# LuoweiZhou/VLP

Measured on NVIDIA H100. Metric: image_text_samples_per_sec, higher is better.
Workload: dtype bf16

## Files before the change

### vlp_b200/csrc/api.cu

```cuda
#include "../../include/vlpk.h"

#include <cstdlib>
#include <cstring>

#include "attn.cuh"
#include "decode.cuh"
#include "gemm.cuh"
#include "head.cuh"
#include "host.cuh"
#include "optim.cuh"
#include "rowops.cuh"
#include "tables.cuh"

using namespace vlpk;
typedef __nv_bfloat16 bf16;

namespace {

inline cudaStream_t S(void* s) { return reinterpret_cast<cudaStream_t>(s); }

enum { SITE_ATTN = 0, SITE_HID1 = 1, SITE_HID2 = 2 };
inline uint64_t site_of(uint64_t layer_id, int site) { return layer_id * 8 + site; }

inline DropoutCfg mk_drop(const VlpkDropout* d, float p, uint64_t site) {
// ... 322 lines not shown
  const long long i = (static_cast<long long>(blockIdx.x) * blockDim.x + threadIdx.x) * 8;
  if (i >= M * N) return;
  const long long r = i / N;
  const int c = static_cast<int>(i % N);
  const uint4 ud = *reinterpret_cast<const uint4*>(dy + r * lddy + c), uy = *reinterpret_cast<const uint4*>(y + r * ldy + c);
  const uint32_t wd[4] = {ud.x, ud.y, ud.z, ud.w}, wy[4] = {uy.x, uy.y, uy.z, uy.w};
  uint32_t o[4];
#pragma unroll
  for (int j = 0; j < 4; ++j) {
    const float2 d = unpack_bf16x2(wd[j]), v = unpack_bf16x2(wy[j]);
    o[j] = pack_bf16x2(v.x > 0.f ? d.x * scale : 0.f, v.y > 0.f ? d.y * scale : 0.f);
  }
  *reinterpret_cast<uint4*>(dpre + i) = make_uint4(o[0], o[1], o[2], o[3]);
}

int score_layer_fwd(const VlpkShape* s, int T, const AttnGroupKv* group, const VlpkLayerWeights* w, const void* x, const uint32_t* key_bits,
                    const uint32_t* query_bits, VlpkLayerActs* a, uint64_t layer_id, cudaStream_t st) {
  const int H = s->H, K = group != nullptr ? T - 1 : s->Lq, R = K + T;
  VLPK_TRY(qkv_fwd(s->B * R, H, w, x, a->qkv, st));
  const bf16* qkv = static_cast<const bf16*>(a->qkv);
  AttnGroupKv g;
  if (group != nullptr) {
    g = *group;
    g.text = qkv + H; g.ld_text = 3 * H; g.T = R; g.pos = 0;
  }
  AttnDesc ad;
  ad.B = s->B; ad.heads = s->heads; ad.Lkv = s->Lkv; ad.kv_slots = s->kv_slots;
  ad.q = qkv; ad.ld_q = 3 * H; ad.q_batch_stride = static_cast<int64_t>(R) * 3 * H;
  ad.k = qkv + H; ad.v = qkv + 2 * H; ad.kv_batch_stride = static_cast<int64_t>(R) * 3 * H;
  ad.ld_kv = group != nullptr ? 2 * H : 3 * H;
  ad.o = a->ctx; ad.ld_o = H; ad.o_batch_stride = static_cast<int64_t>(R) * H;
  ad.lse = a->lse;
  ad.drop = make_dropout(0.f, 0, 0);
  if (K > 0) {
    AttnDesc kd = ad;
    kd.Lq = K;
    kd.mask_bits = key_bits; kd.mask_rows = K;
    VLPK_TRY(launch_attn_fwd(kd, group != nullptr ? &g : nullptr, nullptr, st));
  }
  AttnDesc qd = ad;
  qd.Lq = T;
  qd.q = qkv + static_cast<size_t>(K) * 3 * H;
  qd.o = static_cast<bf16*>(a->ctx) + static_cast<size_t>(K) * H;
  qd.mask_bits = query_bits; qd.mask_rows = T;
  qd.lse = a->lse + static_cast<size_t>(s->B) * s->heads * K;
  AttnSelfKv sk;
  sk.k = qkv + static_cast<size_t>(K) * 3 * H + H;
  sk.v = qkv + static_cast<size_t>(K) * 3 * H + 2 * H;
  sk.ld = 3 * H; sk.batch_stride = static_cast<int64_t>(R) * 3 * H;
  VLPK_TRY(launch_attn_fwd(qd, group != nullptr ? &g : nullptr, &sk, st));
  VlpkShape rows = *s;
  rows.Lq = rows.Lkv = R;
  VLPK_TRY(attn_out_ln(&rows, w, x, a, 0.f, nullptr, layer_id, st));
  return ffn_fwd_impl(&rows, w, a, 0.f, nullptr, layer_id, st);
}

int score_stack_fwd(const VlpkShape* s, int T, int n_layers, const VlpkLayerWeights* w, const void* x, AttnGroupKv* group,
                    const void* const* prefix, const uint32_t* key_bits, const uint32_t* query_bits, VlpkLayerActs* acts, cudaStream_t st) {
  const void* cur = x;
  for (int i = 0; i < n_layers; ++i) {
    if (group != nullptr) group->prefix = prefix[i];
    VLPK_TRY(score_layer_fwd(s, T, group, &w[i], cur, key_bits, query_bits, &acts[i], i, st));
    cur = acts[i].y;
  }
  return 0;
}

size_t act_bytes(const VlpkShape* s, size_t rows, size_t kv_elems) {
  const size_t H = s->H, I = s->I, M = static_cast<size_t>(s->B) * rows;
  const size_t lse = (static_cast<size_t>(s->B) * s->heads * rows + 3) / 4 * 4;
  return 2 * (M * (3 * H + 5 * H + 2 * I) + kv_elems) + 4 * (lse + 4 * M);
}

}

#pragma GCC visibility push(default)
extern "C" {

int vlpk_version(void) { return VLPK_VERSION; }
int vlpk_debug_set_option(const char* name, int value) {
  VLPK_CHECK_ARG(name != nullptr, "set_option: null name");
  if (strcmp(name, "wgrad_stream") == 0) { g_wgrad_stream = value ? 1 : 0; return 0; }
  if (strcmp(name, "attn_tiled") == 0) { set_attn_tiled(value != 0); return 0; }
  set_error("set_option: unknown option '%s'", name);
  return -1;
}
int vlpk_debug_plan_gemm(int M, int N, int K, int a_mn, int b_mn, int nseg, int seg_rows, int epi, int bn, int splits, int* out2) {
  GemmDesc g;
  g.M = M; g.N = N; g.K = K;
  g.a_mn = a_mn != 0; g.b_mn = b_mn != 0;
  g.nseg = nseg; g.b_seg_rows = seg_rows;
  g.epi = epi; g.bn = bn; g.splits = splits;
  return plan_gemm(g, &out2[0], &out2[1]);
}
void vlpk_set_reserved_sms(int n) { set_reserved_sms(n); }
void vlpk_set_deterministic(int on) { set_deterministic(on != 0); }
const char* vlpk_last_error(void) { return get_error(); }

int vlpk_mask_pack(const void* mask, int dtype, int mode, int B, int rows, int kv, int64_t stride_b, int64_t stride_r, uint32_t* out,
                   void* stream) {
  VLPK_CHECK_ARG(mask != nullptr && out != nullptr, "mask_pack: null pointer");
  return launch_mask_pack(mask, dtype, mode, B, rows, kv, stride_b, stride_r, out, S(stream));
}

int vlpk_mask_synth(const int32_t* len_b, const int32_t* mode, int len_a, int B, int L, uint32_t* out, void* stream) {
  return launch_mask_synth(len_b, mode, len_a, B, L, out, S(stream));
}

int vlpk_linear_fwd(int M, int N, int K, const void* x, int64_t ldx, const void* w, int64_t ldw, const void* bias, void* y, int64_t ldy,
                    int act, const VlpkDropout* drop, uint64_t site, void* stream) {
  VLPK_CHECK_ARG(x && w && y, "linear_fwd: null pointer");
  VLPK_CHECK_ARG(act == VLPK_ACT_NONE || act == VLPK_ACT_RELU, "linear_fwd: act %d unsupported", act);
  const DropoutCfg dc = (act == VLPK_ACT_RELU && drop != nullptr) ? mk_drop(drop, drop->p, site) : make_dropout(0.f, 0, site);
  return fwd_linear(M, N, K, x, ldx, w, ldw, bias, y, ldy, act == VLPK_ACT_RELU ? EPI_RELU : EPI_STORE, nullptr, 0, dc, S(stream));
}

int vlpk_linear_bwd(int M, int N, int K, const void* x, int64_t ldx, const void* w, int64_t ldw, const void* y, int64_t ldy,
                    const void* dy, int64_t lddy, void* dpre, void* dx, int64_t lddx, float* dw, int64_t lddw, float* db, int act,
                    float p_drop, void* stream) {
  VLPK_CHECK_ARG(x && w && dy && dw, "linear_bwd: null pointer");
  cudaStream_t st = S(stream);
  const void* g = dy;
  int64_t ldg = lddy;
  if (act == VLPK_ACT_RELU) {
    VLPK_CHECK_ARG(y != nullptr && dpre != nullptr && N % 8 == 0, "linear_bwd: relu needs y, dpre and N %% 8 == 0");
    const long long n = static_cast<long long>(M) * N;
    LaunchScope scope(CAT_MISC, 6.0 * n, st);
    relu_bwd_kernel<<<static_cast<unsigned>((n / 8 + 255) / 256), 256, 0, st>>>(static_cast<bf16*>(dpre), static_cast<const bf16*>(dy),
                                                                             static_cast<const bf16*>(y), M, N, lddy, ldy,
                                                                             p_drop > 0.f ? 1.0f / (1.0f - p_drop) : 1.0f);
    VLPK_CUDA(cudaGetLastError());
    g = dpre;
    ldg = N;
  }
  if (db != nullptr) VLPK_TRY(launch_colsum(g, ldg, M, N, db, st));
  VLPK_TRY(wgrad_linear(M, N, K, g, ldg, x, ldx, dw, lddw, st));
  if (dx != nullptr) VLPK_TRY(dgrad_linear(M, N, K, g, ldg, w, ldw, dx, lddx, EPI_STORE, nullptr, 0, st));
  return 0;
}

static EmbedArgs mk_embed(int B, int L, int H, int R, int vis_input, const int64_t* ids, const int64_t* tt, const int64_t* pos,
                          const void* word_w, const void* pos_w, const void* type_w, const void* vis, const void* vpe,
                          const void* ln_g) {
  EmbedArgs a;
  a.B = B; a.L = L; a.H = H; a.R = R; a.vis_input = vis_input;
  a.ids = reinterpret_cast<const long long*>(ids);
  a.tt = reinterpret_cast<const long long*>(tt);
  a.pos = reinterpret_cast<const long long*>(pos);
  a.word = static_cast<const bf16*>(word_w); a.posw = static_cast<const bf16*>(pos_w); a.typew = static_cast<const bf16*>(type_w);
  a.vis = static_cast<const bf16*>(vis); a.vpe = static_cast<const bf16*>(vpe);
  a.gamma = static_cast<const bf16*>(ln_g);
  return a;
}

int vlpk_embed_fwd(int B, int L, int H, int R, int vis_input, const int64_t* ids, const int64_t* token_type, const int64_t* pos,
                   const void* word_w, const void* pos_w, const void* type_w, const void* vis, const void* vis_pe, const void* ln_g,
                   const void* ln_b, void* y, float* stats, const VlpkDropout* drop, uint64_t site, void* stream) {
  VLPK_CHECK_ARG(ids && word_w && pos_w && type_w && ln_g && ln_b && y, "embed_fwd: null pointer");
  EmbedArgs a = mk_embed(B, L, H, R, vis_input, ids, token_type, pos, word_w, pos_w, type_w, vis, vis_pe, ln_g);
  a.beta = static_cast<const bf16*>(ln_b);
  a.y = static_cast<bf16*>(y);
  a.stats = reinterpret_cast<float2*>(stats);
  a.drop = mk_drop(drop, drop ? drop->p : 0.f, site);
  return launch_embed_fwd(a, S(stream));
}

// ... 476 lines not shown
```

### vlp_b200/csrc/common.cuh

```cuda
#pragma once
#include <cuda.h>
#include <cuda_bf16.h>
#include <cuda_runtime.h>
#include <stdint.h>

#include "wgmma.cuh"

namespace vlpk {

__device__ __forceinline__ uint32_t smem_u32(const void* p) {
  return static_cast<uint32_t>(__cvta_generic_to_shared(p));
}

__device__ __forceinline__ uint32_t lane_id() { return threadIdx.x & 31u; }

__device__ __forceinline__ bool elect_one() {
  uint32_t pred = 0;
  asm volatile(
      "{\n\t"
      ".reg .pred P;\n\t"
      "elect.sync _|P, 0xffffffff;\n\t"
      "selp.u32 %0, 1, 0, P;\n\t"
      "}\n"
      : "=r"(pred));
// ... 4 lines not shown
  asm volatile("mbarrier.init.shared::cta.b64 [%0], %1;" ::"r"(smem_u32(bar)), "r"(count) : "memory");
}
__device__ __forceinline__ void fence_mbar_init() {
  asm volatile("fence.mbarrier_init.release.cluster;" ::: "memory");
}
__device__ __forceinline__ void fence_proxy_async_smem() {
  asm volatile("fence.proxy.async.shared::cta;" ::: "memory");
}
__device__ __forceinline__ void mbar_arrive_expect_tx(uint64_t* bar, uint32_t bytes) {
  asm volatile("mbarrier.arrive.expect_tx.shared::cta.b64 _, [%0], %1;" ::"r"(smem_u32(bar)), "r"(bytes)
               : "memory");
}
__device__ __forceinline__ void mbar_arrive(uint64_t* bar) {
  asm volatile("mbarrier.arrive.shared::cta.b64 _, [%0];" ::"r"(smem_u32(bar)) : "memory");
}
__device__ __forceinline__ bool mbar_try_wait(uint64_t* bar, uint32_t parity) {
  uint32_t ok;
  asm volatile(
      "{\n\t"
      ".reg .pred P;\n\t"
      "mbarrier.try_wait.parity.shared::cta.b64 P, [%1], %2;\n\t"
      "selp.u32 %0, 1, 0, P;\n\t"
      "}\n"
      : "=r"(ok)
      : "r"(smem_u32(bar)), "r"(parity)
      : "memory");
  return ok != 0;
}
__device__ __forceinline__ void mbar_wait(uint64_t* bar, uint32_t parity) {
  uint32_t spins = 0;
  while (!mbar_try_wait(bar, parity)) {
    if (++spins > (1u << 28)) { __trap(); }
  }
}
__device__ __forceinline__ void mbar_wait_flag(uint64_t* bar, uint32_t parity, bool& timed_out) {
  uint32_t spins = 0;
  while (!timed_out && !mbar_try_wait(bar, parity)) {
    if (++spins > (1u << 28)) timed_out = true;
  }
}

__device__ __forceinline__ void pdl_launch_dependents() { asm volatile("griddepcontrol.launch_dependents;" ::: "memory"); }
__device__ __forceinline__ void pdl_wait() { asm volatile("griddepcontrol.wait;" ::: "memory"); }

__device__ __forceinline__ void tma_prefetch_desc(const CUtensorMap* m) {
  asm volatile("prefetch.tensormap [%0];" ::"l"(reinterpret_cast<uint64_t>(m)) : "memory");
}
__device__ __forceinline__ void tma_load_2d(void* dst, const CUtensorMap* m, uint64_t* bar, int c0, int c1) {
  asm volatile(
      "cp.async.bulk.tensor.2d.shared::cluster.global.tile.mbarrier::complete_tx::bytes [%0], [%1, {%3, %4}], [%2];"
      ::"r"(smem_u32(dst)), "l"(reinterpret_cast<uint64_t>(m)), "r"(smem_u32(bar)), "r"(c0), "r"(c1)
      : "memory");
}
__device__ __forceinline__ void tma_load_3d(void* dst, const CUtensorMap* m, uint64_t* bar, int c0, int c1,
                                            int c2) {
  asm volatile(
      "cp.async.bulk.tensor.3d.shared::cluster.global.tile.mbarrier::complete_tx::bytes [%0], [%1, {%3, %4, %5}], "
      "[%2];" ::"r"(smem_u32(dst)),
      "l"(reinterpret_cast<uint64_t>(m)), "r"(smem_u32(bar)), "r"(c0), "r"(c1), "r"(c2)
      : "memory");
}
__device__ __forceinline__ void tma_store_2d(const CUtensorMap* m, const void* src, int c0, int c1) {
  asm volatile("cp.async.bulk.tensor.2d.global.shared::cta.tile.bulk_group [%0, {%2, %3}], [%1];" ::"l"(
                   reinterpret_cast<uint64_t>(m)),
               "r"(smem_u32(src)), "r"(c0), "r"(c1)
               : "memory");
}
__device__ __forceinline__ void tma_store_3d(const CUtensorMap* m, const void* src, int c0, int c1, int c2) {
  asm volatile("cp.async.bulk.tensor.3d.global.shared::cta.tile.bulk_group [%0, {%2, %3, %4}], [%1];" ::"l"(
                   reinterpret_cast<uint64_t>(m)),
               "r"(smem_u32(src)), "r"(c0), "r"(c1), "r"(c2)
               : "memory");
}
__device__ __forceinline__ void tma_reduce_add_2d(const CUtensorMap* m, const void* src, int c0, int c1) {
  asm volatile("cp.reduce.async.bulk.tensor.2d.global.shared::cta.add.tile.bulk_group [%0, {%2, %3}], [%1];" ::"l"(
                   reinterpret_cast<uint64_t>(m)),
               "r"(smem_u32(src)), "r"(c0), "r"(c1)
               : "memory");
}
__device__ __forceinline__ void tma_reduce_add_3d(const CUtensorMap* m, const void* src, int c0, int c1, int c2) {
  asm volatile("cp.reduce.async.bulk.tensor.3d.global.shared::cta.add.tile.bulk_group [%0, {%2, %3, %4}], [%1];" ::"l"(
                   reinterpret_cast<uint64_t>(m)),
               "r"(smem_u32(src)), "r"(c0), "r"(c1), "r"(c2)
               : "memory");
}
__device__ __forceinline__ void tma_store_commit() { asm volatile("cp.async.bulk.commit_group;" ::: "memory"); }
template <int N>
__device__ __forceinline__ void tma_store_wait_read() {
  asm volatile("cp.async.bulk.wait_group.read %0;" ::"n"(N) : "memory");
}
template <int N>
__device__ __forceinline__ void tma_store_wait() {
  asm volatile("cp.async.bulk.wait_group %0;" ::"n"(N) : "memory");
}

__device__ __forceinline__ void wgmma_fence() { asm volatile("wgmma.fence.sync.aligned;" ::: "memory"); }
__device__ __forceinline__ void wgmma_commit() { asm volatile("wgmma.commit_group.sync.aligned;" ::: "memory"); }
template <int N>
__device__ __forceinline__ void wgmma_wait() {
  asm volatile("wgmma.wait_group.sync.aligned %0;" ::"n"(N) : "memory");
}
template <uint32_t N>
__device__ __forceinline__ void setmaxnreg_dec() { asm volatile("setmaxnreg.dec.sync.aligned.u32 %0;" ::"n"(N)); }
template <uint32_t N>
__device__ __forceinline__ void setmaxnreg_inc() { asm volatile("setmaxnreg.inc.sync.aligned.u32 %0;" ::"n"(N)); }
template <int N>
__device__ __forceinline__ void reg_fence(float (&d)[N]) {
#pragma unroll
  for (int i = 0; i < N; ++i) asm volatile("" : "+f"(d[i])::"memory");
}

__device__ __forceinline__ uint64_t wgmma_desc_sw128(uint32_t saddr, uint32_t lbo_bytes, uint32_t sbo_bytes) {
  uint64_t d = 0;
  d |= static_cast<uint64_t>((saddr & 0x3FFFFu) >> 4);
  d |= static_cast<uint64_t>((lbo_bytes >> 4) & 0x3FFFu) << 16;
  d |= static_cast<uint64_t>((sbo_bytes >> 4) & 0x3FFFu) << 32;
  d |= 1ull << 62;
  return d;
}

__device__ __forceinline__ uint32_t pack_bf16x2(float lo, float hi) {
  __nv_bfloat162 v = __floats2bfloat162_rn(lo, hi);
  return *reinterpret_cast<uint32_t*>(&v);
}
__device__ __forceinline__ float2 unpack_bf16x2(uint32_t u) {
  __nv_bfloat162 v = *reinterpret_cast<__nv_bfloat162*>(&u);
  return __bfloat1622float2(v);
}
__device__ __forceinline__ float bf16_round(float x) { return __bfloat162float(__float2bfloat16_rn(x)); }

__device__ __forceinline__ float fast_ex2(float x) {
  float y;
  asm("ex2.approx.ftz.f32 %0, %1;" : "=f"(y) : "f"(x));
  return y;
}
__device__ __forceinline__ float fast_rcp(float x) {
  float y;
  asm("rcp.approx.ftz.f32 %0, %1;" : "=f"(y) : "f"(x));
  return y;
}

__device__ __forceinline__ void gelu_and_grad(float x, float& g, float& d) {
  const float ax = fabsf(x);
  const float e = fast_ex2(-0.72134752044448170f * x * x);
  const float t = fast_rcp(fmaf(0.3275911f * 0.70710678118654752f, ax, 1.0f));
  float poly = fmaf(1.061405429f, t, -1.453152027f);
  poly = fmaf(poly, t, 1.421413741f);
  poly = fmaf(poly, t, -0.284496736f);
  poly = fmaf(poly, t, 0.254829592f);
  poly *= t;
  const float erf_abs = fmaf(-poly, e, 1.0f);
  const float cdf = 0.5f * (1.0f + copysignf(erf_abs, x));
  g = x * cdf;
  d = fmaf(x * 0.3989422804014327f, e, cdf);
}

struct Philox {
  __device__ __forceinline__ static uint4 gen(uint64_t seed, uint64_t ctr_hi, uint64_t ctr_lo) {
    uint32_t k0 = static_cast<uint32_t>(seed), k1 = static_cast<uint32_t>(seed >> 32);
    uint4 c = make_uint4(static_cast<uint32_t>(ctr_lo), static_cast<uint32_t>(ctr_lo >> 32),
                         static_cast<uint32_t>(ctr_hi), static_cast<uint32_t>(ctr_hi >> 32));
#pragma unroll
    for (int i = 0; i < 10; ++i) {
      const uint32_t hi0 = __umulhi(0xD2511F53u, c.x), lo0 = 0xD2511F53u * c.x;
      const uint32_t hi1 = __umulhi(0xCD9E8D57u, c.z), lo1 = 0xCD9E8D57u * c.z;
      c = make_uint4(hi1 ^ c.y ^ k0, lo1, hi0 ^ c.w ^ k1, lo0);
// ... 49 lines not shown
```

### vlp_b200/csrc/rowops.cu

```cuda
#include "rowops.cuh"

#include <cstdlib>
#include "host.cuh"

namespace vlpk {

static constexpr int MAXCH = 4;

__device__ __forceinline__ float warp_sum(float v) {
#pragma unroll
  for (int o = 16; o > 0; o >>= 1) v += __shfl_xor_sync(0xffffffffu, v, o);
  return v;
}

__device__ __forceinline__ void load8(const __nv_bfloat16* p, float (&f)[8]) {
  const uint4 u = __ldg(reinterpret_cast<const uint4*>(p));
  const uint32_t w[4] = {u.x, u.y, u.z, u.w};
#pragma unroll
  for (int j = 0; j < 4; ++j) {
    const float2 x = unpack_bf16x2(w[j]);
    f[2 * j] = x.x;
    f[2 * j + 1] = x.y;
  }
}
__device__ __forceinline__ void store8(__nv_bfloat16* p, const float (&f)[8]) {
  uint4 u;
  u.x = pack_bf16x2(f[0], f[1]);
  u.y = pack_bf16x2(f[2], f[3]);
  u.z = pack_bf16x2(f[4], f[5]);
  u.w = pack_bf16x2(f[6], f[7]);
  *reinterpret_cast<uint4*>(p) = u;
}

template <int NCH>
__device__ __forceinline__ void row_stats(const float (&z)[NCH][8], const bool (&ok)[NCH], int H, float eps,
                                          float& mean, float& rstd) {
  float s = 0.f;
#pragma unroll
  for (int i = 0; i < NCH; ++i)
    if (ok[i]) {
#pragma unroll
      for (int j = 0; j < 8; ++j) s += z[i][j];
    }
  mean = warp_sum(s) / H;
  float v = 0.f;
#pragma unroll
  for (int i = 0; i < NCH; ++i)
    if (ok[i]) {
#pragma unroll
      for (int j = 0; j < 8; ++j) {
        const float d = z[i][j] - mean;
        v += d * d;
      }
    }
  rstd = rsqrtf(warp_sum(v) / H + eps);
}

template <int NCH>
__global__ void __launch_bounds__(256) ln_res_drop_fwd_kernel(LnArgs a) {
  pdl_launch_dependents();
  pdl_wait();
  const uint64_t dseed = drop_seed(a.drop);
  const int lane = threadIdx.x & 31;
  const int wpb = blockDim.x >> 5;
  const long long rowi = static_cast<long long>(blockIdx.x) * wpb + (threadIdx.x >> 5);
  if (rowi >= a.M) return;
  float z[NCH][8];
  bool ok[NCH];
#pragma unroll
  for (int i = 0; i < NCH; ++i) {
    const int col = (lane + 32 * i) * 8;
    ok[i] = col < a.H;
    if (ok[i]) {
      float t[8];
      load8(a.t + rowi * a.H + col, t);
      uint32_t keep = 0xFFu;
      if (a.drop.p > 0.f) keep = dropout_keep8(dseed, a.drop.site, (rowi * a.H + col) >> 3, a.drop.thresh16);
      float r[8] = {0, 0, 0, 0, 0, 0, 0, 0};
      if (a.res != nullptr) load8(a.res + rowi * a.H + col, r);
#pragma unroll
      for (int j = 0; j < 8; ++j) z[i][j] = (((keep >> j) & 1u) ? t[j] * a.drop.scale : 0.f) + r[j];
    }
  }
  float mean, rstd;
  row_stats(z, ok, a.H, a.eps, mean, rstd);
#pragma unroll
  for (int i = 0; i < NCH; ++i) {
    const int col = (lane + 32 * i) * 8;
    if (ok[i]) {
      float g[8], be[8], y[8];
      load8(a.gamma + col, g);
      load8(a.beta + col, be);
#pragma unroll
      for (int j = 0; j < 8; ++j) y[j] = (z[i][j] - mean) * rstd * g[j] + be[j];
      store8(a.y + rowi * a.H + col, y);
    }
  }
  if (lane == 0 && a.stats != nullptr) a.stats[rowi] = make_float2(mean, rstd);
}

static constexpr int LNB_WARPS = 16;

__device__ __forceinline__ int lnb_idx(int i, int half, int lane) { return ((i * 2 + half) * 32 + lane) * 4; }

template <int NCH, bool ORDERED>
__global__ void __launch_bounds__(LNB_WARPS * 32, 1) ln_res_drop_bwd_kernel(LnArgs a) {
  pdl_launch_dependents();
  pdl_wait();
  const uint64_t dseed = drop_seed(a.drop);
  extern __shared__ float s_ln[];
  constexpr int W = NCH * 256;
  const int lane = threadIdx.x & 31;
  const int wib = threadIdx.x >> 5;
  float* sg = s_ln + (wib * 3 + 0) * W;
  float* sb = s_ln + (wib * 3 + 1) * W;
  float* st = s_ln + (wib * 3 + 2) * W;
  float* s_gamma = s_ln + LNB_WARPS * 3 * W;
  bool ok[NCH];
#pragma unroll
  for (int i = 0; i < NCH; ++i) {
    ok[i] = (lane + 32 * i) * 8 < a.H;
#pragma unroll
    for (int h = 0; h < 2; ++h) {
      const float4 z4 = make_float4(0.f, 0.f, 0.f, 0.f);
      *reinterpret_cast<float4*>(sg + lnb_idx(i, h, lane)) = z4;
      *reinterpret_cast<float4*>(sb + lnb_idx(i, h, lane)) = z4;
      *reinterpret_cast<float4*>(st + lnb_idx(i, h, lane)) = z4;
    }
  }
  if (wib == 0) {
#pragma unroll
    for (int i = 0; i < NCH; ++i) {
      float g[8] = {0, 0, 0, 0, 0, 0, 0, 0};
      if (ok[i]) load8(a.gamma + (lane + 32 * i) * 8, g);
      *reinterpret_cast<float4*>(s_gamma + lnb_idx(i, 0, lane)) = make_float4(g[0], g[1], g[2], g[3]);
      *reinterpret_cast<float4*>(s_gamma + lnb_idx(i, 1, lane)) = make_float4(g[4], g[5], g[6], g[7]);
    }
  }
  __syncthreads();

  for (long long rowi = static_cast<long long>(blockIdx.x) * LNB_WARPS + wib; rowi < a.M;
       rowi += static_cast<long long>(gridDim.x) * LNB_WARPS) {
    const float2 stt = a.stats[rowi];
    const float mean = stt.x, rstd = stt.y;
    float xh[NCH][8], gy[NCH][8];
    uint32_t keepm[NCH];
    float s1 = 0.f, s2 = 0.f;
#pragma unroll
    for (int i = 0; i < NCH; ++i) {
      const int col = (lane + 32 * i) * 8;
      keepm[i] = 0xFFu;
      if (ok[i]) {
        float t[8], r[8] = {0, 0, 0, 0, 0, 0, 0, 0}, dy[8];
        load8(a.t + rowi * a.H + col, t);
        if (a.res != nullptr) load8(a.res + rowi * a.H + col, r);
        load8(a.dy + rowi * a.H + col, dy);
        if (a.drop.p > 0.f) keepm[i] = dropout_keep8(dseed, a.drop.site, (rowi * a.H + col) >> 3, a.drop.thresh16);
        float g[8];
        {
          const float4 g0 = *reinterpret_cast<const float4*>(s_gamma + lnb_idx(i, 0, lane));
          const float4 g1 = *reinterpret_cast<const float4*>(s_gamma + lnb_idx(i, 1, lane));
          g[0] = g0.x; g[1] = g0.y; g[2] = g0.z; g[3] = g0.w; g[4] = g1.x; g[5] = g1.y; g[6] = g1.z; g[7] = g1.w;
        }
        float pg[8], pb[8];
#pragma unroll
        for (int j = 0; j < 8; ++j) {
          const float zz = (((keepm[i] >> j) & 1u) ? t[j] * a.drop.scale : 0.f) + r[j];
          xh[i][j] = (zz - mean) * rstd;
          gy[i][j] = dy[j] * g[j];
          s1 += gy[i][j];
          s2 += gy[i][j] * xh[i][j];
          pg[j] = dy[j] * xh[i][j];
          pb[j] = dy[j];
        }
#pragma unroll
        for (int h = 0; h < 2; ++h) {
          float4* pgs = reinterpret_cast<float4*>(sg + lnb_idx(i, h, lane));
          float4* pbs = reinterpret_cast<float4*>(sb + lnb_idx(i, h, lane));
          float4 vg = *pgs, vb = *pbs;
          vg.x += pg[4 * h]; vg.y += pg[4 * h + 1]; vg.z += pg[4 * h + 2]; vg.w += pg[4 * h + 3];
          vb.x += pb[4 * h]; vb.y += pb[4 * h + 1]; vb.z += pb[4 * h + 2]; vb.w += pb[4 * h + 3];
          *pgs = vg;
          *pbs = vb;
        }
      }
    }
    const float c1 = warp_sum(s1) / a.H, c2 = warp_sum(s2) / a.H;
#pragma unroll
    for (int i = 0; i < NCH; ++i) {
      const int col = (lane + 32 * i) * 8;
      if (ok[i]) {
        float dz[8], dt[8];
#pragma unroll
        for (int j = 0; j < 8; ++j) {
          dz[j] = rstd * (gy[i][j] - c1 - xh[i][j] * c2);
          dt[j] = ((keepm[i] >> j) & 1u) ? dz[j] * a.drop.scale : 0.f;
        }
        if (a.dz != nullptr) store8(a.dz + rowi * a.H + col, dz);
        if (a.dt != nullptr) store8(a.dt + rowi * a.H + col, dt);
        if (a.dbias != nullptr) {
#pragma unroll
          for (int h = 0; h < 2; ++h) {
            float4* pts = reinterpret_cast<float4*>(st + lnb_idx(i, h, lane));
            float4 vt = *pts;
            vt.x += dt[4 * h]; vt.y += dt[4 * h + 1]; vt.z += dt[4 * h + 2]; vt.w += dt[4 * h + 3];
            *pts = vt;
          }
        }
      }
    }
  }
  __syncthreads();
  for (int c = threadIdx.x; c < a.H; c += blockDim.x) {
    const int idx = lnb_idx(c >> 8, (c & 7) >> 2, (c & 255) >> 3) + (c & 3);
    float vg = 0.f, vb = 0.f, vt = 0.f;
#pragma unroll 4
    for (int w = 0; w < LNB_WARPS; ++w) {
      vg += s_ln[(w * 3 + 0) * W + idx];
      vb += s_ln[(w * 3 + 1) * W + idx];
      vt += s_ln[(w * 3 + 2) * W + idx];
    }
    if constexpr (ORDERED) {
      const long long slab = static_cast<long long>(gridDim.x) * a.H, o = static_cast<long long>(blockIdx.x) * a.H + c;
      if (a.dgamma != nullptr) a.part[o] = vg;
      if (a.dbeta != nullptr) a.part[slab + o] = vb;
      if (a.dbias != nullptr) a.part[2 * slab + o] = vt;
    } else {
      if (a.dgamma != nullptr) atomicAdd(a.dgamma + c, vg);
      if (a.dbeta != nullptr) atomicAdd(a.dbeta + c, vb);
      if (a.dbias != nullptr) atomicAdd(a.dbias + c, vt);
    }
  }
}

#define VLPK_DISPATCH_NCH(H, ...)                  \
  do {                                             \
    const int _nch = ((H) + 255) / 256;            \
    if (_nch == 1) { constexpr int NCH = 1; __VA_ARGS__; }      \
    else if (_nch == 2) { constexpr int NCH = 2; __VA_ARGS__; } \
    else if (_nch == 3) { constexpr int NCH = 3; __VA_ARGS__; } \
    else { constexpr int NCH = 4; __VA_ARGS__; }   \
  } while (0)

static inline bool misaligned(const void* p, unsigned mask) { return (reinterpret_cast<uintptr_t>(p) & mask) != 0; }

static int check_ln(const LnArgs& a) {
  VLPK_CHECK_ARG(a.M > 0 && a.H > 0 && a.H % 8 == 0 && a.H <= MAXCH * 256, "layernorm: H=%d must be a multiple of 8 and <= %d",
                 a.H, MAXCH * 256);
  VLPK_CHECK_ARG(!(misaligned(a.t, 15) || misaligned(a.res, 15) || misaligned(a.gamma, 15) || misaligned(a.beta, 15) || misaligned(a.y, 15) ||
                   misaligned(a.dy, 15) || misaligned(a.dz, 15) || misaligned(a.dt, 15) || misaligned(a.stats, 7) ||
                   misaligned(a.dgamma, 3) || misaligned(a.dbeta, 3) || misaligned(a.dbias, 3)),
                 "layernorm: bf16 buffers must be 16-byte aligned (stats 8, fp32 accumulators 4)");
  return 0;
}

int launch_ln_res_drop_fwd(const LnArgs& a, cudaStream_t s) {
  VLPK_TRY(check_ln(a));
  const int wpb = 8;
  const long long grid = (a.M + wpb - 1) / wpb;
  LaunchScope scope(CAT_LN_FWD, 2.0 * a.M * a.H * (a.res ? 3 : 2) + 8.0 * a.M, s);
  VLPK_DISPATCH_NCH(a.H, VLPK_CUDA(launch_ex(ln_res_drop_fwd_kernel<NCH>, dim3(static_cast<unsigned>(grid)), dim3(wpb * 32), 0, s, 1, a)));
  return 0;
}

int launch_ln_res_drop_bwd(const LnArgs& a, cudaStream_t s) {
  VLPK_TRY(check_ln(a));
  VLPK_CHECK_ARG(a.dy != nullptr && a.stats != nullptr, "layernorm bwd: missing dy / stats");
  const int nch = (a.H + 255) / 256;
  long long grid = (a.M + LNB_WARPS - 1) / LNB_WARPS;
  if (grid > num_sms()) grid = num_sms();
  const size_t smem = static_cast<size_t>(LNB_WARPS * 3 + 1) * nch * 256 * sizeof(float);
  static bool attr_set = false;
  if (!attr_set) {
    VLPK_CUDA(cudaFuncSetAttribute(ln_res_drop_bwd_kernel<1, false>, cudaFuncAttributeMaxDynamicSharedMemorySize, (LNB_WARPS * 3 + 1) * 1 * 1024));
    VLPK_CUDA(cudaFuncSetAttribute(ln_res_drop_bwd_kernel<2, false>, cudaFuncAttributeMaxDynamicSharedMemorySize, (LNB_WARPS * 3 + 1) * 2 * 1024));
    VLPK_CUDA(cudaFuncSetAttribute(ln_res_drop_bwd_kernel<3, false>, cudaFuncAttributeMaxDynamicSharedMemorySize, (LNB_WARPS * 3 + 1) * 3 * 1024));
    VLPK_CUDA(cudaFuncSetAttribute(ln_res_drop_bwd_kernel<4, false>, cudaFuncAttributeMaxDynamicSharedMemorySize, (LNB_WARPS * 3 + 1) * 4 * 1024));
    VLPK_CUDA(cudaFuncSetAttribute(ln_res_drop_bwd_kernel<1, true>, cudaFuncAttributeMaxDynamicSharedMemorySize, (LNB_WARPS * 3 + 1) * 1 * 1024));
    VLPK_CUDA(cudaFuncSetAttribute(ln_res_drop_bwd_kernel<2, true>, cudaFuncAttributeMaxDynamicSharedMemorySize, (LNB_WARPS * 3 + 1) * 2 * 1024));
    VLPK_CUDA(cudaFuncSetAttribute(ln_res_drop_bwd_kernel<3, true>, cudaFuncAttributeMaxDynamicSharedMemorySize, (LNB_WARPS * 3 + 1) * 3 * 1024));
    VLPK_CUDA(cudaFuncSetAttribute(ln_res_drop_bwd_kernel<4, true>, cudaFuncAttributeMaxDynamicSharedMemorySize, (LNB_WARPS * 3 + 1) * 4 * 1024));
    attr_set = true;
  }
  if (!deterministic()) {
    LaunchScope scope(CAT_LN_BWD, 2.0 * a.M * a.H * ((a.res ? 3 : 2) + (a.dz ? 1 : 0) + (a.dt ? 1 : 0)) + 8.0 * a.M, s);
    VLPK_DISPATCH_NCH(a.H, VLPK_CUDA(launch_ex(ln_res_drop_bwd_kernel<NCH, false>, dim3(static_cast<unsigned>(grid)), dim3(LNB_WARPS * 32), smem, s, 1, a)));
    return 0;
  }
  const long long n = grid * a.H;
  LnArgs b = a;
  b.part = scratch_f32(SCRATCH_ORDERED, static_cast<size_t>(3 * n), s);
  if (b.part == nullptr) return -1;
  {
    LaunchScope scope(CAT_LN_BWD, 2.0 * a.M * a.H * ((a.res ? 3 : 2) + (a.dz ? 1 : 0) + (a.dt ? 1 : 0)) + 8.0 * a.M, s);
    VLPK_DISPATCH_NCH(a.H, VLPK_CUDA(launch_ex(ln_res_drop_bwd_kernel<NCH, true>, dim3(static_cast<unsigned>(grid)), dim3(LNB_WARPS * 32), smem, s, 1, b)));
  }
  float* outs[3] = {a.dgamma, a.dbeta, a.dbias};
  for (int k = 0; k < 3; ++k)
    if (outs[k] != nullptr) VLPK_TRY(launch_sum_parts(b.part + k * n, static_cast<int>(grid), a.H, outs[k], s));
  return 0;
}

template <int NCH>
__device__ __forceinline__ void embed_row_z(const EmbedArgs& a, long long rowi, int lane, float (&z)[NCH][8], bool (&ok)[NCH]) {
  const int b = static_cast<int>(rowi / a.L), l = static_cast<int>(rowi % a.L);
  const bool vis = a.vis_input && l >= 1 && l <= a.R;
  const long long wid = a.ids[rowi];
  const long long pid = a.pos != nullptr ? a.pos[rowi] : l;
  const long long tid = a.tt != nullptr ? a.tt[rowi] : 0;
  const __nv_bfloat16* wsrc = vis ? a.vis + (static_cast<long long>(b) * a.R + (l - 1)) * a.H : a.word + wid * a.H;
  const __nv_bfloat16* psrc = vis ? a.vpe + (static_cast<long long>(b) * a.R + (l - 1)) * a.H : a.posw + pid * a.H;
  const __nv_bfloat16* tsrc = a.typew + tid * a.H;
#pragma unroll
  for (int i = 0; i < NCH; ++i) {
    const int col = (lane + 32 * i) * 8;
    ok[i] = col < a.H;
    if (ok[i]) {
      float w[8], p[8], t[8];
      load8(wsrc + col, w);
      load8(psrc + col, p);
      load8(tsrc + col, t);
#pragma unroll
      for (int j = 0; j < 8; ++j) z[i][j] = w[j] + p[j] + t[j];
    }
  }
}

template <int NCH>
__global__ void __launch_bounds__(256) embed_fwd_kernel(EmbedArgs a) {
  const uint64_t dseed = drop_seed(a.drop);
  const int lane = threadIdx.x & 31;
  const int wpb = blockDim.x >> 5;
  const long long rowi = static_cast<long long>(blockIdx.x) * wpb + (threadIdx.x >> 5);
  const long long M = static_cast<long long>(a.B) * a.L;
  if (rowi >= M) return;
  float z[NCH][8];
  bool ok[NCH];
  embed_row_z(a, rowi, lane, z, ok);
  float mean, rstd;
  row_stats(z, ok, a.H, a.eps, mean, rstd);
#pragma unroll
  for (int i = 0; i < NCH; ++i) {
    const int col = (lane + 32 * i) * 8;
    if (ok[i]) {
      float g[8], be[8], y[8];
      load8(a.gamma + col, g);
      load8(a.beta + col, be);
      uint32_t keep = 0xFFu;
      if (a.drop.p > 0.f) keep = dropout_keep8(dseed, a.drop.site, (rowi * a.H + col) >> 3, a.drop.thresh16);
#pragma unroll
      for (int j = 0; j < 8; ++j) {
        const float v = (z[i][j] - mean) * rstd * g[j] + be[j];
        y[j] = ((keep >> j) & 1u) ? v * a.drop.scale : 0.f;
      }
      store8(a.y + rowi * a.H + col, y);
    }
  }
  if (lane == 0 && a.stats != nullptr) a.stats[rowi] = make_float2(mean, rstd);
}

template <int NCH, bool ORDERED>
__global__ void __launch_bounds__(256) embed_bwd_kernel(EmbedArgs a) {
  const uint64_t dseed = drop_seed(a.drop);
  extern __shared__ float s_red[];
  const int lane = threadIdx.x & 31;
  const int wib = threadIdx.x >> 5;
  const int wpb = blockDim.x >> 5;
  const long long M = static_cast<long long>(a.B) * a.L;
  float ag[NCH][8], ab[NCH][8], g[NCH][8];
  bool okc[NCH];
#pragma unroll
  for (int i = 0; i < NCH; ++i) {
    okc[i] = (lane + 32 * i) * 8 < a.H;
    if (okc[i]) load8(a.gamma + (lane + 32 * i) * 8, g[i]);
#pragma unroll
    for (int j = 0; j < 8; ++j) ag[i][j] = ab[i][j] = 0.f;
  }
  for (long long rowi = static_cast<long long>(blockIdx.x) * wpb + wib; rowi < M;
// ... 338 lines not shown
```

### vlp_b200/csrc/rowops.cuh

```cuda
#pragma once
#include "common.cuh"

namespace vlpk {

enum { VLPK_DT_BF16 = 0, VLPK_DT_F32 = 1, VLPK_DT_I64 = 2 };
enum { MASK_ADDITIVE = 0, MASK_ZERO_ONE = 1 };

struct LnArgs {
  long long M = 0;
  int H = 0;
  float eps = 1e-5f;
  const __nv_bfloat16* t = nullptr;
  const __nv_bfloat16* res = nullptr;
  const __nv_bfloat16* gamma = nullptr;
  const __nv_bfloat16* beta = nullptr;
  __nv_bfloat16* y = nullptr;
  float2* stats = nullptr;
  DropoutCfg drop = {0.f, 1.f, 0u, 0ull, 0ull, nullptr};
  const __nv_bfloat16* dy = nullptr;
  __nv_bfloat16* dz = nullptr;
  __nv_bfloat16* dt = nullptr;
  float* dgamma = nullptr;
  float* dbeta = nullptr;
  float* dbias = nullptr;
  float* part = nullptr;
};

int launch_ln_res_drop_fwd(const LnArgs& a, cudaStream_t s);
int launch_ln_res_drop_bwd(const LnArgs& a, cudaStream_t s);

struct EmbedArgs {
  int B = 0, L = 0, H = 0, R = 0;
  int vis_input = 1;
  float eps = 1e-5f;
  const long long* ids = nullptr;
  const long long* tt = nullptr;
  const long long* pos = nullptr;
  const __nv_bfloat16* word = nullptr;
  const __nv_bfloat16* posw = nullptr;
  const __nv_bfloat16* typew = nullptr;
  const __nv_bfloat16* vis = nullptr;
  const __nv_bfloat16* vpe = nullptr;
  const __nv_bfloat16* gamma = nullptr;
  const __nv_bfloat16* beta = nullptr;
  __nv_bfloat16* y = nullptr;
  float2* stats = nullptr;
  DropoutCfg drop = {0.f, 1.f, 0u, 0ull, 0ull, nullptr};
  const __nv_bfloat16* dy = nullptr;
  __nv_bfloat16* dz = nullptr;
  float* dgamma = nullptr;
  float* dbeta = nullptr;
  float* part = nullptr;
};

int launch_embed_fwd(const EmbedArgs& a, cudaStream_t s);
int launch_embed_bwd(const EmbedArgs& a, cudaStream_t s);

int launch_mask_pack(const void* mask, int dtype, int mode, int B, int rows, int kv, long long stride_b, long long stride_r,
                     uint32_t* out, cudaStream_t s);
int launch_mask_synth(const int* len_b, const int* mode, int len_a, int B, int L, uint32_t* out, cudaStream_t s);
int launch_colsum(const void* x, long long ld, long long M, int N, float* out, cudaStream_t s);
int launch_sum_parts(const float* part, int parts, long long n, float* out, cudaStream_t s);
int launch_f32_to_bf16(const float* x, void* y, long long n, cudaStream_t s);
int launch_dropout_mask(const DropoutCfg& d, long long n, unsigned char* out, cudaStream_t s);


}
```

Before: 5380.

## Prefetch layernorm-backward row inputs via bulk async copies into per-warp smem ring

```diff
diff --git a/vlp_b200/csrc/api.cu b/vlp_b200/csrc/api.cu
--- a/vlp_b200/csrc/api.cu
+++ b/vlp_b200/csrc/api.cu
@@ -428,6 +428,7 @@
   VLPK_CHECK_ARG(name != nullptr, "set_option: null name");
   if (strcmp(name, "wgrad_stream") == 0) { g_wgrad_stream = value ? 1 : 0; return 0; }
   if (strcmp(name, "attn_tiled") == 0) { set_attn_tiled(value != 0); return 0; }
+  if (strcmp(name, "ln_grid") == 0) { set_ln_grid_cap(value); return 0; }
   set_error("set_option: unknown option '%s'", name);
   return -1;
 }
diff --git a/vlp_b200/csrc/common.cuh b/vlp_b200/csrc/common.cuh
--- a/vlp_b200/csrc/common.cuh
+++ b/vlp_b200/csrc/common.cuh
@@ -110,6 +110,11 @@
   asm volatile("cp.reduce.async.bulk.tensor.3d.global.shared::cta.add.tile.bulk_group [%0, {%2, %3, %4}], [%1];" ::"l"(
                    reinterpret_cast<uint64_t>(m)),
                "r"(smem_u32(src)), "r"(c0), "r"(c1), "r"(c2)
+               : "memory");
+}
+__device__ __forceinline__ void bulk_load(void* dst, const void* src, uint32_t bytes, uint64_t* bar) {
+  asm volatile("cp.async.bulk.shared::cluster.global.mbarrier::complete_tx::bytes [%0], [%1], %2, [%3];" ::"r"(smem_u32(dst)),
+               "l"(reinterpret_cast<uint64_t>(src)), "r"(bytes), "r"(smem_u32(bar))
                : "memory");
 }
 __device__ __forceinline__ void tma_store_commit() { asm volatile("cp.async.bulk.commit_group;" ::: "memory"); }
diff --git a/vlp_b200/csrc/rowops.cu b/vlp_b200/csrc/rowops.cu
--- a/vlp_b200/csrc/rowops.cu
+++ b/vlp_b200/csrc/rowops.cu
@@ -99,23 +99,64 @@
   if (lane == 0 && a.stats != nullptr) a.stats[rowi] = make_float2(mean, rstd);
 }
 
-static constexpr int LNB_WARPS = 16;
+static constexpr int LN_BAR_BYTES = 8;
+
+static int g_ln_grid_cap = 0;
+void set_ln_grid_cap(int n) { g_ln_grid_cap = n > 0 ? n : 0; }
+static long long ln_grid(long long grid) { return (g_ln_grid_cap > 0 && grid > g_ln_grid_cap) ? g_ln_grid_cap : grid; }
+
+__device__ __forceinline__ void lds8(const __nv_bfloat16* p, float (&f)[8]) {
+  const uint4 u = *reinterpret_cast<const uint4*>(p);
+  const uint32_t w[4] = {u.x, u.y, u.z, u.w};
+#pragma unroll
+  for (int j = 0; j < 4; ++j) {
+    const float2 x = unpack_bf16x2(w[j]);
+    f[2 * j] = x.x;
+    f[2 * j + 1] = x.y;
+  }
+}
+
+__device__ __forceinline__ void ln_request(const LnArgs& a, long long rowi, const __nv_bfloat16* a0, const __nv_bfloat16* a1,
+                                           const __nv_bfloat16* a2, __nv_bfloat16* dst, uint64_t* bar) {
+  if (rowi >= a.M) return;
+  const uint32_t bytes = static_cast<uint32_t>(a.H) * 2u;
+  mbar_arrive_expect_tx(bar, bytes * (1u + (a1 != nullptr) + (a2 != nullptr)));
+  bulk_load(dst, a0 + rowi * a.H, bytes, bar);
+  if (a1 != nullptr) bulk_load(dst + a.H, a1 + rowi * a.H, bytes, bar);
+  if (a2 != nullptr) bulk_load(dst + 2 * a.H, a2 + rowi * a.H, bytes, bar);
+}
+
+template <int NCH>
+struct LnbCfg {
+  static constexpr int WARPS = NCH == 4 ? 8 : 16;
+  static constexpr int STAGES = NCH == 3 ? 1 : 2;
+};
+
+template <int NCH>
+static size_t lnb_smem(int H) {
+  return static_cast<size_t>(LnbCfg<NCH>::WARPS * 3 + 1) * NCH * 256 * sizeof(float) +
+         static_cast<size_t>(LnbCfg<NCH>::WARPS) * LnbCfg<NCH>::STAGES * (LN_BAR_BYTES + 3 * H * 2);
+}
 
 __device__ __forceinline__ int lnb_idx(int i, int half, int lane) { return ((i * 2 + half) * 32 + lane) * 4; }
 
 template <int NCH, bool ORDERED>
-__global__ void __launch_bounds__(LNB_WARPS * 32, 1) ln_res_drop_bwd_kernel(LnArgs a) {
-  pdl_launch_dependents();
-  pdl_wait();
-  const uint64_t dseed = drop_seed(a.drop);
-  extern __shared__ float s_ln[];
+__global__ void __launch_bounds__(LnbCfg<NCH>::WARPS * 32, 1) ln_res_drop_bwd_kernel(LnArgs a) {
+  constexpr int LNB_WARPS = LnbCfg<NCH>::WARPS;
+  constexpr int STAGES = LnbCfg<NCH>::STAGES;
   constexpr int W = NCH * 256;
+  extern __shared__ __align__(16) float s_ln[];
   const int lane = threadIdx.x & 31;
   const int wib = threadIdx.x >> 5;
   float* sg = s_ln + (wib * 3 + 0) * W;
   float* sb = s_ln + (wib * 3 + 1) * W;
   float* st = s_ln + (wib * 3 + 2) * W;
   float* s_gamma = s_ln + LNB_WARPS * 3 * W;
+  uint64_t* bar = reinterpret_cast<uint64_t*>(s_gamma + W) + wib * STAGES;
+  __nv_bfloat16* ring = reinterpret_cast<__nv_bfloat16*>(reinterpret_cast<uint64_t*>(s_gamma + W) + LNB_WARPS * STAGES) +
+                        static_cast<size_t>(wib) * STAGES * 3 * a.H;
+  const long long stride = static_cast<long long>(gridDim.x) * LNB_WARPS;
+  const long long row0 = static_cast<long long>(blockIdx.x) * LNB_WARPS + wib;
   bool ok[NCH];
 #pragma unroll
   for (int i = 0; i < NCH; ++i) {
@@ -128,6 +169,16 @@
       *reinterpret_cast<float4*>(st + lnb_idx(i, h, lane)) = z4;
     }
   }
+  if (lane == 0) {
+    for (int s = 0; s < STAGES; ++s) mbar_init(&bar[s], 1);
+    fence_mbar_init();
+  }
+  __syncwarp();
+  pdl_launch_dependents();
+  pdl_wait();
+  if (lane == 0)
+    for (int s = 0; s < STAGES; ++s) ln_request(a, row0 + s * stride, a.t, a.dy, a.res, ring + s * 3 * a.H, &bar[s]);
+  const uint64_t dseed = drop_seed(a.drop);
   if (wib == 0) {
 #pragma unroll
     for (int i = 0; i < NCH; ++i) {
@@ -139,10 +190,16 @@
   }
   __syncthreads();
 
-  for (long long rowi = static_cast<long long>(blockIdx.x) * LNB_WARPS + wib; rowi < a.M;
-       rowi += static_cast<long long>(gridDim.x) * LNB_WARPS) {
-    const float2 stt = a.stats[rowi];
+  bool timed_out = false;
+  int s = 0;
+  uint32_t phase = 0;
+  float2 stt_next = row0 < a.M ? a.stats[row0] : make_float2(0.f, 0.f);
+  for (long long rowi = row0; rowi < a.M; rowi += stride) {
+    const float2 stt = stt_next;
+    if (rowi + stride < a.M) stt_next = a.stats[rowi + stride];
     const float mean = stt.x, rstd = stt.y;
+    mbar_wait_flag(&bar[s], phase, timed_out);
+    const __nv_bfloat16* sr = ring + s * 3 * a.H;
     float xh[NCH][8], gy[NCH][8];
     uint32_t keepm[NCH];
     float s1 = 0.f, s2 = 0.f;
@@ -152,9 +209,9 @@
       keepm[i] = 0xFFu;
       if (ok[i]) {
         float t[8], r[8] = {0, 0, 0, 0, 0, 0, 0, 0}, dy[8];
-        load8(a.t + rowi * a.H + col, t);
-        if (a.res != nullptr) load8(a.res + rowi * a.H + col, r);
-        load8(a.dy + rowi * a.H + col, dy);
+        lds8(sr + col, t);
+        if (a.res != nullptr) lds8(sr + 2 * a.H + col, r);
+        lds8(sr + a.H + col, dy);
         if (a.drop.p > 0.f) keepm[i] = dropout_keep8(dseed, a.drop.site, (rowi * a.H + col) >> 3, a.drop.thresh16);
         float g[8];
         {
@@ -185,6 +242,12 @@
         }
       }
     }
+    __syncwarp();
+    if (lane == 0) ln_request(a, rowi + STAGES * stride, a.t, a.dy, a.res, ring + s * 3 * a.H, &bar[s]);
+    if (++s == STAGES) {
+      s = 0;
+      phase ^= 1u;
+    }
     const float c1 = warp_sum(s1) / a.H, c2 = warp_sum(s2) / a.H;
 #pragma unroll
     for (int i = 0; i < NCH; ++i) {
@@ -210,11 +273,12 @@
       }
     }
   }
+  if (timed_out) __trap();
   __syncthreads();
   for (int c = threadIdx.x; c < a.H; c += blockDim.x) {
     const int idx = lnb_idx(c >> 8, (c & 7) >> 2, (c & 255) >> 3) + (c & 3);
     float vg = 0.f, vb = 0.f, vt = 0.f;
-#pragma unroll 4
+#pragma unroll
     for (int w = 0; w < LNB_WARPS; ++w) {
       vg += s_ln[(w * 3 + 0) * W + idx];
       vb += s_ln[(w * 3 + 1) * W + idx];
@@ -266,25 +330,24 @@
 int launch_ln_res_drop_bwd(const LnArgs& a, cudaStream_t s) {
   VLPK_TRY(check_ln(a));
   VLPK_CHECK_ARG(a.dy != nullptr && a.stats != nullptr, "layernorm bwd: missing dy / stats");
-  const int nch = (a.H + 255) / 256;
-  long long grid = (a.M + LNB_WARPS - 1) / LNB_WARPS;
+  int warps = 0;
+  size_t smem = 0;
+  VLPK_DISPATCH_NCH(a.H, (warps = LnbCfg<NCH>::WARPS, smem = lnb_smem<NCH>(a.H)));
+  long long grid = (a.M + warps - 1) / warps;
   if (grid > num_sms()) grid = num_sms();
-  const size_t smem = static_cast<size_t>(LNB_WARPS * 3 + 1) * nch * 256 * sizeof(float);
+  grid = ln_grid(grid);
   static bool attr_set = false;
   if (!attr_set) {
-    VLPK_CUDA(cudaFuncSetAttribute(ln_res_drop_bwd_kernel<1, false>, cudaFuncAttributeMaxDynamicSharedMemorySize, (LNB_WARPS * 3 + 1) * 1 * 1024));
-    VLPK_CUDA(cudaFuncSetAttribute(ln_res_drop_bwd_kernel<2, false>, cudaFuncAttributeMaxDynamicSharedMemorySize, (LNB_WARPS * 3 + 1) * 2 * 1024));
-    VLPK_CUDA(cudaFuncSetAttribute(ln_res_drop_bwd_kernel<3, false>, cudaFuncAttributeMaxDynamicSharedMemorySize, (LNB_WARPS * 3 + 1) * 3 * 1024));
-    VLPK_CUDA(cudaFuncSetAttribute(ln_res_drop_bwd_kernel<4, false>, cudaFuncAttributeMaxDynamicSharedMemorySize, (LNB_WARPS * 3 + 1) * 4 * 1024));
-    VLPK_CUDA(cudaFuncSetAttribute(ln_res_drop_bwd_kernel<1, true>, cudaFuncAttributeMaxDynamicSharedMemorySize, (LNB_WARPS * 3 + 1) * 1 * 1024));
-    VLPK_CUDA(cudaFuncSetAttribute(ln_res_drop_bwd_kernel<2, true>, cudaFuncAttributeMaxDynamicSharedMemorySize, (LNB_WARPS * 3 + 1) * 2 * 1024));
-    VLPK_CUDA(cudaFuncSetAttribute(ln_res_drop_bwd_kernel<3, true>, cudaFuncAttributeMaxDynamicSharedMemorySize, (LNB_WARPS * 3 + 1) * 3 * 1024));
-    VLPK_CUDA(cudaFuncSetAttribute(ln_res_drop_bwd_kernel<4, true>, cudaFuncAttributeMaxDynamicSharedMemorySize, (LNB_WARPS * 3 + 1) * 4 * 1024));
+#define VLPK_LNB_ATTR(N)                                                                                                            \
+    VLPK_CUDA(cudaFuncSetAttribute(ln_res_drop_bwd_kernel<N, false>, cudaFuncAttributeMaxDynamicSharedMemorySize, static_cast<int>(lnb_smem<N>(N * 256)))); \
+    VLPK_CUDA(cudaFuncSetAttribute(ln_res_drop_bwd_kernel<N, true>, cudaFuncAttributeMaxDynamicSharedMemorySize, static_cast<int>(lnb_smem<N>(N * 256))));
+    VLPK_LNB_ATTR(1) VLPK_LNB_ATTR(2) VLPK_LNB_ATTR(3) VLPK_LNB_ATTR(4)
+#undef VLPK_LNB_ATTR
     attr_set = true;
   }
   if (!deterministic()) {
     LaunchScope scope(CAT_LN_BWD, 2.0 * a.M * a.H * ((a.res ? 3 : 2) + (a.dz ? 1 : 0) + (a.dt ? 1 : 0)) + 8.0 * a.M, s);
-    VLPK_DISPATCH_NCH(a.H, VLPK_CUDA(launch_ex(ln_res_drop_bwd_kernel<NCH, false>, dim3(static_cast<unsigned>(grid)), dim3(LNB_WARPS * 32), smem, s, 1, a)));
+    VLPK_DISPATCH_NCH(a.H, VLPK_CUDA(launch_ex(ln_res_drop_bwd_kernel<NCH, false>, dim3(static_cast<unsigned>(grid)), dim3(warps * 32), smem, s, 1, a)));
     return 0;
   }
   const long long n = grid * a.H;
@@ -293,7 +356,7 @@
   if (b.part == nullptr) return -1;
   {
     LaunchScope scope(CAT_LN_BWD, 2.0 * a.M * a.H * ((a.res ? 3 : 2) + (a.dz ? 1 : 0) + (a.dt ? 1 : 0)) + 8.0 * a.M, s);
-    VLPK_DISPATCH_NCH(a.H, VLPK_CUDA(launch_ex(ln_res_drop_bwd_kernel<NCH, true>, dim3(static_cast<unsigned>(grid)), dim3(LNB_WARPS * 32), smem, s, 1, b)));
+    VLPK_DISPATCH_NCH(a.H, VLPK_CUDA(launch_ex(ln_res_drop_bwd_kernel<NCH, true>, dim3(static_cast<unsigned>(grid)), dim3(warps * 32), smem, s, 1, b)));
   }
   float* outs[3] = {a.dgamma, a.dbeta, a.dbias};
   for (int k = 0; k < 3; ++k)
diff --git a/vlp_b200/csrc/rowops.cuh b/vlp_b200/csrc/rowops.cuh
--- a/vlp_b200/csrc/rowops.cuh
+++ b/vlp_b200/csrc/rowops.cuh
@@ -28,6 +28,7 @@
 
 int launch_ln_res_drop_fwd(const LnArgs& a, cudaStream_t s);
 int launch_ln_res_drop_bwd(const LnArgs& a, cudaStream_t s);
+void set_ln_grid_cap(int n);
 
 struct EmbedArgs {
   int B = 0, L = 0, H = 0, R = 0;
```

Result: no change. 5365 (median of 6 runs) (-0.3%).
